# ZihaoW123/UniMM

Hardware: AMD Instinct MI355X
Metric: dialog-sequences/sec (fwd+bwd) at bs=240 seq=256 regions=36(+1 <IMG>) (higher is better)
Workload: dtype bf16; 1 GPU; UniMM-UL sparse training step (BASELINE configs[1]): bert_base_6layer_6conect, sequences_per_image=6, num_negative_samples=5, mask_prob=0.15, dropout on, MLM+UL / NSP / region-KL losses, fwd+bwd, optimizer step not included; global_batch=240, per_gpu_batch=240, seq_len=256, regions=37, parallelism=dp1, executor=eager launches, step_api=loss = combine(losses); loss.backward() (autograd, as train.py:164-168, :315)

## Files before the change

### include/unimm_hip.h

```cpp
#ifndef UNIMM_HIP_H
#define UNIMM_HIP_H

#include <stdint.h>

#ifdef __cplusplus
extern "C" {
#endif

#define UNIMM_OK 0
#define UNIMM_E_ARG (-1)
#define UNIMM_E_SHAPE (-2)
#define UNIMM_E_ALIGN (-3)
#define UNIMM_E_HIP (-4)

int unimm_version(void);
const char* unimm_arch(void);

enum {
  UNIMM_EPI_BIAS = 0,
  UNIMM_EPI_BIAS_GELU = 1,
  UNIMM_EPI_BIAS_DROP_RESID = 2,
  UNIMM_EPI_BIAS_RELU = 3,
  UNIMM_EPI_DGELU = 4,
  UNIMM_EPI_ADD = 5,
// ... 61 lines not shown
  const int32_t* order;
} unimm_attn_args;

int unimm_attn_fwd(const unimm_attn_args* args, void* stream);

int unimm_attn_probs(const unimm_attn_args* args, float* probs, void* stream);

typedef struct {
  const void* q; const void* k; const void* v; const void* out; const void* dout;
  const float* lse; float* delta;
  void* dq; void* dk; void* dv;
  const uint32_t* mask;
  const int32_t* q_off; const int32_t* q_len; const int32_t* k_off; const int32_t* k_len;
  int32_t B, H, Tq, Tk, D;
  int32_t ldq, ldk, ldv, ldo, lddo, lddq, lddk, lddv;
  int32_t mask_q_stride, mask_b_stride;
  float scale;
  uint32_t drop_key, drop_thr; float drop_scale;
  const uint32_t* drop_salt;
  const int32_t* order;
} unimm_attn_bwd_args;

int unimm_attn_bwd(const unimm_attn_bwd_args* args, void* stream);

enum { UNIMM_DT_U8 = 0, UNIMM_DT_I32 = 1, UNIMM_DT_I64 = 2, UNIMM_DT_F32 = 3 };

int unimm_mask_pack(const void* mask, int dtype, uint32_t* out, int64_t rows, int32_t t, void* stream);
int unimm_host_mask_pack(const void* mask, int dtype, uint32_t* out, int64_t rows, int32_t t, int32_t threads);
int unimm_host_memcpy(void* dst, const void* src, int64_t bytes, int32_t threads);
int unimm_mask_synth(const int32_t* mode, const int32_t* len, const int32_t* nans, uint32_t* text_words, uint32_t* co_words,
                     int32_t B, int32_t T, void* stream);

int unimm_plan_lengths(const uint32_t* text_words, int32_t t_q_stride, int32_t t_b_stride, const uint32_t* co_words,
                       int32_t c_q_stride, int32_t c_b_stride, int32_t R, const int32_t* labels, const int32_t* weights,
                       const float* nsp_weight, const int32_t* image_label, int32_t B, int32_t T, int32_t* header,
                       void* stream);
int unimm_plan_build(const int32_t* header, const int32_t* labels, const int32_t* weights, int32_t B, int32_t T,
                     int32_t* off, int32_t* lens, int64_t* rows, int64_t* inv, int32_t* lm_pos, int32_t* lm_idx,
                     int32_t* lm_label, int32_t* lm_weight, int32_t rows_cap, int32_t lm_cap, int32_t* dims_i, float* dims_f,
                     int32_t* order, void* stream);

int unimm_layernorm_fwd(const float* x, const float* gamma, const float* beta, float* y32, void* y16, float* mean,
                        float* rstd, int32_t M, int32_t H, float eps, uint32_t drop_key, uint32_t drop_thr,
                        float drop_scale, const uint32_t* drop_salt, void* stream);

int64_t unimm_colpartials_bytes(int32_t H);
// ... 210 lines not shown
```

### unimm_amd/csrc/api.hip

```cpp
#include "common.h"

extern "C" int unimm_version(void) { return 19; }
extern "C" const char* unimm_arch(void) { return "gfx950"; }
```

### unimm_amd/csrc/attention.hip

```cpp
#include <type_traits>
#include "common.h"

namespace {

struct AttnParams {
  const bf16_t* q; const bf16_t* k; const bf16_t* v;
  bf16_t* o; float* lse;
  const uint32_t* mask;
  const int* q_off; const int* q_len; const int* k_off; const int* k_len;
  const int* ks_off; const int* ks_len; int ks_ins;
  const int* order;
  int B, H, Tq, Tk, ldq, ldk, ldv, ldo;
  int mask_q_stride, mask_b_stride;
  int parts;
  float scale;
  DropoutArg drop;
};

constexpr float LOG2E = 1.4426950408889634f;
constexpr float LN2 = 0.6931471805599453f;

template <int D> __device__ __forceinline__ int swz(int row) {
  if constexpr (D == 64) { const int t = row >> 1; return (t & 7) ^ ((t & 1) << 2); }
  else return ((row & 3) << 2) | ((row >> 2) & 3);
// ... 58 lines not shown

__device__ __forceinline__ bf16x8 pack8(const float* p) {
  typedef __attribute__((ext_vector_type(4))) unsigned int u4;
  u4 w = {pack2bf(p[0], p[1]), pack2bf(p[2], p[3]), pack2bf(p[4], p[5]), pack2bf(p[6], p[7])};
  return __builtin_bit_cast(bf16x8, w);
}

__device__ __forceinline__ int key_of_reg(int reg, int h) { return (reg & 3) + 8 * (reg >> 2) + 4 * h; }

template <int D>
__device__ __forceinline__ void store_acc_row(bf16_t* __restrict__ g, const f32x16 (&a)[D / 32], float s, int h, bool ok) {
#pragma unroll
  for (int dt = 0; dt < D / 32; ++dt)
#pragma unroll
    for (int qp = 0; qp < 2; ++qp) {
      const uint32_t a0 = pack2bf(a[dt][8 * qp] * s, a[dt][8 * qp + 1] * s), a1 = pack2bf(a[dt][8 * qp + 2] * s, a[dt][8 * qp + 3] * s);
      const uint32_t b0 = pack2bf(a[dt][8 * qp + 4] * s, a[dt][8 * qp + 5] * s), b1 = pack2bf(a[dt][8 * qp + 6] * s, a[dt][8 * qp + 7] * s);
      const auto w0 = __builtin_amdgcn_permlane32_swap(a0, b0, false, false);
      const auto w1 = __builtin_amdgcn_permlane32_swap(a1, b1, false, false);
      if (ok) *reinterpret_cast<u32x4*>(g + 32 * dt + 16 * qp + 8 * h) = u32x4{w0[0], w1[0], w0[1], w1[1]};
    }
}

template <int D, int NKT>
__global__ __launch_bounds__(512, 2) void attn_fwd_kernel(AttnParams p) {
  drop_resolve(p.drop);
  extern __shared__ __attribute__((aligned(16))) char smem[];
  constexpr int KPAD = NKT * 32;
  char* kimg = smem;
  char* vimg = smem + KPAD * 2 * D;
  const int tid = threadIdx.x, wave = tid >> 6, lane = tid & 63;
  const int item = blockIdx.x / p.parts, part = blockIdx.x % p.parts;
  const int b = p.order != nullptr ? p.order[item / p.H] : item / p.H, head = item % p.H;
  const int nwv = blockDim.x >> 6;
  const int r = lane & 31, h = lane >> 5;

  const int Ts_b = p.ks_len ? p.ks_len[b] : 0;
  int Tk_b = (p.k_len ? p.k_len[b] : p.Tk) + Ts_b;
  Tk_b = Tk_b < KPAD ? Tk_b : KPAD;
  const int Tq_b = p.q_len ? p.q_len[b] : p.Tq;
  if (part * (int)(blockDim.x >> 6) * 32 >= Tq_b) return;
  const size_t qbase = p.q_off ? (size_t)p.q_off[b] : (size_t)b * p.Tq;
  const size_t kbase = p.k_off ? (size_t)p.k_off[b] : (size_t)b * p.Tk;
  const size_t sbase = p.ks_off ? (size_t)p.ks_off[b] : 0;
  const int kpad_b = ((Tk_b + 31) & ~31) < KPAD ? ((Tk_b + 31) & ~31) : KPAD;
  stage_head_seg<D>(p.k + head * D, p.ldk, kbase, sbase, p.ks_ins, Ts_b, Tk_b, kpad_b, kimg, tid, blockDim.x);
  stage_head_seg<D>(p.v + head * D, p.ldv, kbase, sbase, p.ks_ins, Ts_b, Tk_b, kpad_b, vimg, tid, blockDim.x);

  int wt = part * nwv + wave;
  int q0, qrow;
  bool qvalid;
  bf16x8 qf[D / 16];
  uint32_t mw[NKT];
#define UNIMM_LOAD_QTILE()                                                                                    \
  {                                                                                                          \
    q0 = wt * 32;                                                                                            \
    qrow = q0 + r;                                                                                           \
    qvalid = qrow < Tq_b;                                                                                    \
    if (!qvalid) qrow = Tq_b - 1;                                                                            \
    const bf16_t* qg_ = p.q + (qbase + qrow) * p.ldq + head * D;                                             \
    _Pragma("unroll") for (int ks = 0; ks < D / 16; ++ks) qf[ks] = *reinterpret_cast<const bf16x8*>(qg_ + 16 * ks + 8 * h); \
    const uint32_t* mp_ = p.mask + (size_t)b * p.mask_b_stride + (size_t)qrow * p.mask_q_stride;            \
    _Pragma("unroll") for (int t = 0; t < NKT; ++t) mw[t] = 32 * t < p.Tk ? mp_[t] : 0u;    \
  }
  UNIMM_LOAD_QTILE()
  stage_wait();
  __syncthreads();
  constexpr bool WALK = D == 64;
  for (bool first = true; wt * 32 < Tq_b && (WALK || first); first = false, wt += nwv * p.parts) {
    if (WALK && !first) UNIMM_LOAD_QTILE()

  f32x16 s[NKT];
#pragma unroll
  for (int t = 0; t < NKT; ++t) {
    f32x16 acc = {};
    if (32 * t < Tk_b) {
#pragma unroll
      for (int ks = 0; ks < D / 16; ++ks) {
        const bf16x8 kf = read_row_frag<D>(kimg, 32 * t + r, 2 * ks + h);
        acc = __builtin_amdgcn_mfma_f32_32x32x16_bf16(kf, qf[ks], acc, 0, 0, 0);
      }
    }
    s[t] = acc;
  }

  const float c1 = p.scale * LOG2E;
  constexpr float MOFF = -10000.0f * LOG2E;
  int tk_here = Tk_b;
  asm volatile("" : "+v"(tk_here));
  float mx = -INFINITY;
// ... 56 lines not shown
  for (int dt = 0; dt < D / 32; ++dt) o[dt] = f32x16{};
#pragma unroll
  for (int t = 0; t < NKT; ++t) {
    if (32 * t >= Tk_b) continue;
#pragma unroll
    for (int ss = 0; ss < 2; ++ss) {
      float pv[8];
#pragma unroll
      for (int j = 0; j < 8; ++j) pv[j] = s[t][8 * ss + j];
      const bf16x8 pf = pack8(pv);
#pragma unroll
      for (int dt = 0; dt < D / 32; ++dt) {
        const bf16x8 vf = read_tr_frag<D>(vimg, 32 * t + 16 * ss, 32 * dt, lane);
        o[dt] = __builtin_amdgcn_mfma_f32_32x32x16_bf16(vf, pf, o[dt], 0, 0, 0);
      }
    }
  }

  store_acc_row<D>(p.o + (qbase + (qvalid ? qrow : 0)) * p.ldo + head * D, o, inv, h, qvalid);
  if (qvalid) {
    if (p.lse != nullptr && h == 0) p.lse[((size_t)b * p.H + head) * p.Tq + qrow] = (mx + __log2f(sum)) * LN2;
  }
  }
#undef UNIMM_LOAD_QTILE
}


struct AttnBwdParams {
  const bf16_t* q; const bf16_t* k; const bf16_t* v; const bf16_t* o; const bf16_t* dout;
  const float* lse; float* delta;
  bf16_t* dq; bf16_t* dk; bf16_t* dv;
  const uint32_t* mask;
  const int* q_off; const int* q_len; const int* k_off; const int* k_len;
  const int* order;
  int B, H, Tq, Tk, ldq, ldk, ldv, ldo, lddo, lddq, lddk, lddv;
  int mask_q_stride, mask_b_stride;
  int parts;
  float scale;
  DropoutArg drop;
};

template <int D, int NKT>
__global__ __launch_bounds__(512, 2) void attn_bwd_dq_kernel(AttnBwdParams p) {
  drop_resolve(p.drop);
  extern __shared__ __attribute__((aligned(16))) char smem[];
  constexpr int KPAD = NKT * 32;
// ... 517 lines not shown
        const u32x2 hi = *reinterpret_cast<const u32x2*>(tile + r * 64 + (((4 * ss + 2 + h) ^ tile64_swz(r)) << 3));
        const bf16x8 pf = __builtin_bit_cast(bf16x8, u32x4{lo[0], lo[1], hi[0], hi[1]});
        const bf16x8 vf = read_tr_frag<D>(vimg, 32 * t + 16 * ss, 32 * dt, lane);
        o1[0] = __builtin_amdgcn_mfma_f32_32x32x16_bf16(vf, pf, o1[0], 0, 0, 0);
      }
    }
    float mx = -INFINITY, sum = 0.f;
#pragma unroll
    for (int w = 0; w < NW; ++w) {
      mx = fmaxf(mx, mx_w[w * QPAD + 32 * qt2 + r]);
      sum += sm_w[w * QPAD + 32 * qt2 + r];
    }
    const float inv = (p.drop.thr != 0u ? p.drop.scale : 1.0f) / sum;
    const int q = 32 * qt2 + r;
    const bool qvalid = q < Tq_b;
    store_acc_row<32>(p.o + (qbase + (qvalid ? q : 0)) * p.ldo + head * D + 32 * dt, o1, inv, h, qvalid);
    if (dt == 0 && qvalid && h == 0 && p.lse != nullptr) p.lse[((size_t)b * p.H + head) * p.Tq + q] = (mx + __log2f(sum)) * LN2;
  }
}

template <int NQT>
__global__ __launch_bounds__(512, 2) void attn_bwd_fused_kernel(AttnBwdParams p) {
  constexpr int D = 64;
  drop_resolve(p.drop);
  extern __shared__ __attribute__((aligned(16))) char smem[];
  constexpr int QPAD = NQT * 32;
  constexpr int AS = D + 4;
  char* qimg = smem;
  char* doimg = smem + QPAD * 2 * D;
  float* lse_s = reinterpret_cast<float*>(smem + 2 * QPAD * 2 * D);
  float* del_s = lse_s + QPAD;
  uint32_t* mw_s = reinterpret_cast<uint32_t*>(del_s + QPAD);
  char* scr = reinterpret_cast<char*>(mw_s + 8 * QPAD);
  float* acc = reinterpret_cast<float*>(scr + 8 * 2048);
  int* turn = reinterpret_cast<int*>(acc + QPAD * AS);
  const int tid = threadIdx.x, wave = tid >> 6, lane = tid & 63;
  const int item = blockIdx.x;
  const int b = p.order != nullptr ? p.order[item / p.H] : item / p.H, head = item % p.H;
  const int wt = wave;
  const int r = lane & 31, h = lane >> 5;

  const int Tq_b = p.q_len ? p.q_len[b] : p.Tq, Tk_b = p.k_len ? p.k_len[b] : p.Tk;
  const size_t qbase = p.q_off ? (size_t)p.q_off[b] : (size_t)b * p.Tq;
  const size_t kbase = p.k_off ? (size_t)p.k_off[b] : (size_t)b * p.Tk;
  const int qpad_b = ((Tq_b + 31) & ~31) < QPAD ? ((Tq_b + 31) & ~31) : QPAD;
  stage_head<D>(p.q + qbase * p.ldq + head * D, p.ldq, Tq_b, qpad_b, qimg, tid, blockDim.x);
// ... 10 lines not shown
  const bf16_t* vg = p.v + grow * p.ldv + head * D;
  bf16x8 kf[D / 16], vf[D / 16];
#pragma unroll
  for (int ks = 0; ks < D / 16; ++ks) {
    kf[ks] = *reinterpret_cast<const bf16x8*>(kg + 16 * ks + 8 * h);
    vf[ks] = *reinterpret_cast<const bf16x8*>(vg + 16 * ks + 8 * h);
  }
  bf16x8 ktf[2][2];
  {
    char* kt = reinterpret_cast<char*>(acc) + wave * (32 * 2 * D);
#pragma unroll
    for (int ks = 0; ks < D / 16; ++ks) {
      const u32x4 v = kvalid ? __builtin_bit_cast(u32x4, kf[ks]) : u32x4{0u, 0u, 0u, 0u};
      *reinterpret_cast<u32x4*>(kt + r * (2 * D) + (((2 * ks + h) ^ swz<D>(r)) << 4)) = v;
    }
#pragma unroll
    for (int ss = 0; ss < 2; ++ss) {
      ktf[0][ss] = read_tr_frag<D>(kt, 16 * ss, 0, lane);
      ktf[1][ss] = read_tr_frag<D>(kt, 16 * ss, 32, lane);
    }
  }
  stage_wait();
  __syncthreads();

  f32x16 dk[D / 32], dv[D / 32];
#pragma unroll
  for (int dt = 0; dt < D / 32; ++dt) { dk[dt] = f32x16{}; dv[dt] = f32x16{}; }
  const uint32_t* mrow = mw_s + wt * QPAD;
  char* ws = scr + wave * 2048;
  const uint32_t hbase = ((uint32_t)b * p.H + head) * (uint32_t)p.Tq;
  const uint32_t halfw = ((uint32_t)p.Tk + 1u) >> 1, halfm = halfw * DROP_M1;
  const uint32_t dlane = drop_lin(p.drop, (4u * (uint32_t)h + ((uint32_t)r & 1u)) * halfw + ((uint32_t)(wt * 32 + r) >> 1));
  const float c1 = p.scale * LOG2E;
  const bool dropping = p.drop.thr != 0u;
  const uint32_t thr16 = dropping ? (p.drop.thr >> 16) : 0u;
  const float dsc = dropping ? p.drop.scale : 1.0f;
  const BwdScoreCtx sctx{dlane, hbase, halfm, thr16, dsc, c1, dropping};

  if (wave_on) {
#pragma unroll 1
  for (int qt = 0; qt < NQT; ++qt) {
    if (32 * qt >= Tq_b) break;
    f32x16 sacc = {}, dpacc = {};
#pragma unroll
    for (int ks = 0; ks < D / 16; ++ks) {
      const bf16x8 qf = read_row_frag<D>(qimg, 32 * qt + r, 2 * ks + h);
// ... 34 lines not shown
        for (int g = 0; g < 4; ++g)
          *reinterpret_cast<f32x4*>(ap + 32 * dt + 8 * g) = f32x4{dqp[dt][4 * g], dqp[dt][4 * g + 1], dqp[dt][4 * g + 2], dqp[dt][4 * g + 3]};
    } else {
      while (__hip_atomic_load(turn + qt, __ATOMIC_ACQUIRE, __HIP_MEMORY_SCOPE_WORKGROUP) != wt) __builtin_amdgcn_s_sleep(2);
#pragma unroll
      for (int dt = 0; dt < 2; ++dt)
#pragma unroll
        for (int g = 0; g < 4; ++g) {
          f32x4* a4 = reinterpret_cast<f32x4*>(ap + 32 * dt + 8 * g);
          const f32x4 o = *a4;
          *a4 = f32x4{o[0] + dqp[dt][4 * g], o[1] + dqp[dt][4 * g + 1], o[2] + dqp[dt][4 * g + 2], o[3] + dqp[dt][4 * g + 3]};
        }
    }
    if (lane == 0) __hip_atomic_store(turn + qt, wt + 1, __ATOMIC_RELEASE, __HIP_MEMORY_SCOPE_WORKGROUP);
  }
  }

  if (wave_on) {
    const bool ok = kvalid;
    store_acc_row<D>(p.dk + (ok ? grow : 0) * p.lddk + head * D, dk, p.scale, h, ok);
    store_acc_row<D>(p.dv + (ok ? grow : 0) * p.lddv + head * D, dv, 1.0f, h, ok);
  }
  __syncthreads();
  for (int i = tid; i < qpad_b * 8; i += blockDim.x) {
    const int q = i >> 3, c = i & 7;
    if (q >= Tq_b) continue;
    float v[8];
#pragma unroll
    for (int j = 0; j < 8; ++j) v[j] = acc[q * AS + 8 * c + j] * p.scale;
    *reinterpret_cast<u32x4*>(p.dq + (qbase + q) * p.lddq + head * D + 8 * c) =
        u32x4{pack2bf(v[0], v[1]), pack2bf(v[2], v[3]), pack2bf(v[4], v[5]), pack2bf(v[6], v[7])};
  }
}

template <int NQT>
__global__ __launch_bounds__(512, 2) void attn_bwd_fewq128_kernel(AttnBwdParams p) {
  constexpr int D = 128;
  static_assert(NQT == 2, "the (sequence, head) item's queries are two 32-row tiles: P / dS of both stay in registers for phase 2");
  drop_resolve(p.drop);
  extern __shared__ __attribute__((aligned(16))) char smem[];
  constexpr int QPAD = NQT * 32;
  char* qimg = smem;
  char* doimg = smem + QPAD * 2 * D;
  float* lse_s = reinterpret_cast<float*>(smem + 2 * QPAD * 2 * D);
  float* del_s = lse_s + QPAD;
  uint32_t* mw_s = reinterpret_cast<uint32_t*>(del_s + QPAD);
  char* scr = reinterpret_cast<char*>(mw_s + 8 * QPAD);
  char* kimgs = scr + 8 * NQT * 2048;
  const int tid = threadIdx.x, wave = tid >> 6, lane = tid & 63;
  const int item = blockIdx.x;
  const int b = p.order != nullptr ? p.order[item / p.H] : item / p.H, head = item % p.H;
  const int wt = wave;
  const int r = lane & 31, h = lane >> 5;

// ... 313 lines not shown
    }
  }
  auto kern = attn_bwd_dkv_kernel<D, NQT>;
  if (set_lds(kern, lds) != UNIMM_OK) return UNIMM_E_HIP;
  hipLaunchKernelGGL(kern, dim3(p.B * p.H * q.parts), dim3(block_threads((tiles + q.parts - 1) / q.parts, NQT * 32)), lds, s, q);
  UNIMM_CHECK_LAUNCH();
  return UNIMM_OK;
}

template <int NQT>
int launch_bwd_fused(const AttnBwdParams& p, hipStream_t s) {
  constexpr int D = 64, QPAD = NQT * 32;
  const size_t lds = (size_t)2 * QPAD * 2 * D + 2 * QPAD * sizeof(float) + (size_t)8 * QPAD * sizeof(uint32_t) + 8 * 2048 +
                     (size_t)QPAD * (D + 4) * sizeof(float) + NQT * sizeof(int);
  auto kern = attn_bwd_fused_kernel<NQT>;
  if (set_lds(kern, lds) != UNIMM_OK) return UNIMM_E_HIP;
  AttnBwdParams q = p;
  q.parts = 1;
  hipLaunchKernelGGL(kern, dim3(p.B * p.H), dim3(512), lds, s, q);
  UNIMM_CHECK_LAUNCH();
  return UNIMM_OK;
}

inline int launch_bwd_fewq128(const AttnBwdParams& p, hipStream_t s) {
  constexpr int D = 128, NQT = 2, QPAD = NQT * 32;
  const size_t lds = (size_t)2 * QPAD * 2 * D + 2 * QPAD * sizeof(float) + (size_t)8 * QPAD * sizeof(uint32_t) + 8 * NQT * 2048 +
                     (size_t)8 * 32 * 2 * D;
  auto kern = attn_bwd_fewq128_kernel<NQT>;
  if (set_lds(kern, lds) != UNIMM_OK) return UNIMM_E_HIP;
  AttnBwdParams q = p;
  q.parts = 1;
  hipLaunchKernelGGL(kern, dim3(p.B * p.H), dim3(512), lds, s, q);
  UNIMM_CHECK_LAUNCH();
  return UNIMM_OK;
}

inline int launch_bwd_fewk128(const AttnBwdParams& p, hipStream_t s) {
  constexpr int D = 128, KPAD = 64, QMAX = 256;
  const size_t lds = (size_t)2 * KPAD * 2 * D + 2 * QMAX * sizeof(float) + (size_t)2 * QMAX * sizeof(uint32_t) + 8 * 6144 +
                     (size_t)2 * (QMAX / 32) * 2 * 2 * 1024;
  auto kern = attn_bwd_fewk128_kernel;
  if (set_lds(kern, lds) != UNIMM_OK) return UNIMM_E_HIP;
  AttnBwdParams q = p;
  q.parts = 1;
  hipLaunchKernelGGL(kern, dim3(p.B * p.H), dim3(512), lds, s, q);
  UNIMM_CHECK_LAUNCH();
// ... 69 lines not shown
  }
#pragma unroll
  for (int o = 32; o > 0; o >>= 1) mx = fmaxf(mx, __shfl_xor(mx, o, 64));
  float sum = 0.f;
#pragma unroll
  for (int j = 0; j < 4; ++j) {
    sc[j] = (lane + 64 * j) < p.Tk ? __expf(sc[j] - mx) : 0.f;
    sum += sc[j];
  }
  sum = wave_sum(sum);
  const float inv = 1.0f / sum;
  float* out = probs + (size_t)row * p.Tk;
#pragma unroll
  for (int j = 0; j < 4; ++j) {
    const int key = lane + 64 * j;
    if (key >= p.Tk) continue;
    float v = sc[j] * inv;
    if (p.drop.thr != 0u) v = drop_apply(p.drop, (uint32_t)row, (uint32_t)p.Tk, (uint32_t)key, v);
    out[key] = v;
  }
}

}

extern "C" int unimm_attn_fwd(const unimm_attn_args* a, void* stream) {
  if (a == nullptr || !a->q || !a->k || !a->v || !a->out || !a->mask) return UNIMM_E_ARG;
  if (a->B <= 0 || a->H <= 0 || a->Tq <= 0 || a->Tk <= 0 || a->Tq > 256 || a->Tk > 256) return UNIMM_E_SHAPE;
  if (a->D != 64 && a->D != 128) return UNIMM_E_SHAPE;
  if ((a->ldq % 8) || (a->ldk % 8) || (a->ldv % 8) || (a->ldo % 8)) return UNIMM_E_ALIGN;
  if (((uintptr_t)a->q | (uintptr_t)a->k | (uintptr_t)a->v | (uintptr_t)a->out) & 15) return UNIMM_E_ALIGN;
  AttnParams p;
  p.q = (const bf16_t*)a->q; p.k = (const bf16_t*)a->k; p.v = (const bf16_t*)a->v;
  p.o = (bf16_t*)a->out; p.lse = a->lse; p.mask = a->mask;
  p.q_off = a->q_off; p.q_len = a->q_len; p.k_off = a->k_off; p.k_len = a->k_len;
  if ((p.q_off == nullptr) != (p.q_len == nullptr) || (p.k_off == nullptr) != (p.k_len == nullptr)) return UNIMM_E_ARG;
  p.ks_off = a->ks_off; p.ks_len = a->ks_len; p.ks_ins = a->ks_ins;
  if ((p.ks_off == nullptr) != (p.ks_len == nullptr)) return UNIMM_E_ARG;
  if (p.ks_off != nullptr && (p.k_off == nullptr || a->ks_ins < 0 || a->drop_thr != 0u)) return UNIMM_E_ARG;
  if (p.ks_off == nullptr) p.ks_ins = 0;
  p.order = a->order;
  p.B = a->B; p.H = a->H; p.Tq = a->Tq; p.Tk = a->Tk;
  p.ldq = a->ldq; p.ldk = a->ldk; p.ldv = a->ldv; p.ldo = a->ldo;
  p.mask_q_stride = a->mask_q_stride; p.mask_b_stride = a->mask_b_stride;
  p.scale = a->scale;
  p.drop.key = a->drop_key; p.drop.thr = a->drop_thr; p.drop.scale = a->drop_scale; p.drop.salt = a->drop_salt;
  hipStream_t s = (hipStream_t)stream;
// ... 34 lines not shown
  if (a->B <= 0 || a->H <= 0 || a->Tq <= 0 || a->Tk <= 0 || a->Tq > 256 || a->Tk > 256) return UNIMM_E_SHAPE;
  if (a->D != 64 && a->D != 128) return UNIMM_E_SHAPE;
  if ((a->ldq % 8) || (a->ldk % 8) || (a->ldv % 8) || (a->ldo % 8) || (a->lddo % 8) || (a->lddq % 8) || (a->lddk % 8) ||
      (a->lddv % 8))
    return UNIMM_E_ALIGN;
  if (((uintptr_t)a->q | (uintptr_t)a->k | (uintptr_t)a->v | (uintptr_t)a->out | (uintptr_t)a->dout | (uintptr_t)a->dq |
       (uintptr_t)a->dk | (uintptr_t)a->dv) & 15)
    return UNIMM_E_ALIGN;
  AttnBwdParams p;
  p.q = (const bf16_t*)a->q; p.k = (const bf16_t*)a->k; p.v = (const bf16_t*)a->v; p.o = (const bf16_t*)a->out;
  p.dout = (const bf16_t*)a->dout; p.lse = a->lse; p.delta = a->delta;
  p.dq = (bf16_t*)a->dq; p.dk = (bf16_t*)a->dk; p.dv = (bf16_t*)a->dv; p.mask = a->mask;
  p.q_off = a->q_off; p.q_len = a->q_len; p.k_off = a->k_off; p.k_len = a->k_len;
  if ((p.q_off == nullptr) != (p.q_len == nullptr) || (p.k_off == nullptr) != (p.k_len == nullptr)) return UNIMM_E_ARG;
  p.order = a->order;
  p.B = a->B; p.H = a->H; p.Tq = a->Tq; p.Tk = a->Tk;
  p.ldq = a->ldq; p.ldk = a->ldk; p.ldv = a->ldv; p.ldo = a->ldo; p.lddo = a->lddo;
  p.lddq = a->lddq; p.lddk = a->lddk; p.lddv = a->lddv;
  p.mask_q_stride = a->mask_q_stride; p.mask_b_stride = a->mask_b_stride;
  p.scale = a->scale;
  p.drop.key = a->drop_key; p.drop.thr = a->drop_thr; p.drop.scale = a->drop_scale; p.drop.salt = a->drop_salt;
  hipStream_t s = (hipStream_t)stream;
  const bool small_k = a->Tk <= 64, small_q = a->Tq <= 64;
  if (a->D == 64 && !small_k && !small_q) return launch_bwd_fused<8>(p, s);
#ifndef UNIMM_ATTN_FEWQ128
#define UNIMM_ATTN_FEWQ128 1
#endif
  if (UNIMM_ATTN_FEWQ128 && a->D == 128 && small_q && !small_k) return launch_bwd_fewq128(p, s);
#ifndef UNIMM_ATTN_FEWK128
#define UNIMM_ATTN_FEWK128 1
#endif
  if (UNIMM_ATTN_FEWK128 && a->D == 128 && small_k && !small_q) return launch_bwd_fewk128(p, s);
  int rc;
  if (a->D == 64) rc = small_k ? launch_bwd_dq<64, 2>(p, s) : launch_bwd_dq<64, 8>(p, s);
  else rc = small_k ? launch_bwd_dq<128, 2>(p, s) : launch_bwd_dq<128, 8>(p, s);
  if (rc != UNIMM_OK) return rc;
  if (a->D == 64) return small_q ? launch_bwd_dkv<64, 2>(p, s) : launch_bwd_dkv<64, 8>(p, s);
  return small_q ? launch_bwd_dkv<128, 2>(p, s) : launch_bwd_dkv<128, 8>(p, s);
}
```

### unimm_amd/lib.py

```python
from __future__ import annotations

import ctypes as C
import os
import threading

import torch

_PKG = os.path.dirname(os.path.abspath(__file__))
LIB_PATH = os.path.join(_PKG, "libunimm_hip.so")
ABI_VERSION = 19

EPI_BIAS, EPI_BIAS_GELU, EPI_BIAS_DROP_RESID, EPI_BIAS_RELU, EPI_DGELU, EPI_ADD, EPI_MUL, EPI_BIAS_GELU_DG = range(8)

_ERR = {-1: "UNIMM_E_ARG", -2: "UNIMM_E_SHAPE", -3: "UNIMM_E_ALIGN", -4: "UNIMM_E_HIP"}


class UnimmHipError(RuntimeError):
    pass


class GemmNtArgs(C.Structure):
    _fields_ = [("x", C.c_void_p), ("w", C.c_void_p), ("bias", C.c_void_p), ("aux", C.c_void_p),
                ("out", C.c_void_p), ("out2", C.c_void_p),
                ("M", C.c_int32), ("N", C.c_int32), ("K", C.c_int32),
                ("ldx", C.c_int32), ("ldw", C.c_int32), ("ldaux", C.c_int32), ("ldo", C.c_int32),
                ("epilogue", C.c_int32), ("out_f32", C.c_int32),
                ("drop_key", C.c_uint32), ("drop_thr", C.c_uint32), ("drop_scale", C.c_float),
                ("aux_mean", C.c_void_p), ("aux_rstd", C.c_void_p), ("aux_gamma", C.c_void_p), ("aux_beta", C.c_void_p),
                ("tile", C.c_int32), ("drop_salt", C.c_void_p),
                ("splitk_ws", C.c_void_p), ("splitk_ws_bytes", C.c_int64), ("splitk", C.c_int32)]


class GemmTnArgs(C.Structure):
# ... 37 lines not shown
    L.unimm_kv_cache_update.argtypes = [VP, VP]
    L.unimm_lm_topk.argtypes = [VP, I32, I32, I32, VP, I32, VP, I32, I32, VP, VP, VP, VP]
    L.unimm_gemm_tn_grouped.argtypes = [VP, I32, VP]
    L.unimm_gemm_tn_grouped_ws.argtypes = [VP, I32, I32, VP, I64, VP]
    L.unimm_colpartials_finish_grouped.argtypes = [VP, I32, VP]
    L.unimm_layernorm_fwd.argtypes = [VP] * 7 + [I32, I32, F32, U32, U32, F32, VP, VP]
    L.unimm_x3_layernorm_fwd.argtypes = [VP] * 7 + [I32, I32, F32, U32, U32, F32, VP, VP]
    L.unimm_layernorm_bwd_partials.argtypes = [VP] * 8 + [I32, I32, U32, U32, F32, U32, U32, F32, VP, VP, VP, VP]
    L.unimm_layernorm_bwd.argtypes = [VP] * 11 + [I32, I32, U32, U32, F32, U32, U32, F32, VP, VP]
    _lib = L
    return L


SYMBOLS = ["unimm_version", "unimm_arch", "unimm_gemm_nt", "unimm_gemm_tn", "unimm_gemm_tn_grouped", "unimm_attn_fwd", "unimm_attn_bwd",
           "unimm_mask_pack", "unimm_layernorm_fwd", "unimm_colpartials_bytes", "unimm_layernorm_bwd",
           "unimm_embed_fwd", "unimm_embed_bwd", "unimm_colsum", "unimm_cast_f32_bf16", "unimm_transpose_cast",
           "unimm_pack_image", "unimm_mul_dropout", "unimm_mul_dropout_bwd", "unimm_lm_loss_fwd",
           "unimm_lm_loss_bwd", "unimm_kl_loss_fwd", "unimm_kl_loss_bwd", "unimm_nsp_loss_fwd",
           "unimm_nsp_loss_bwd", "unimm_reduce_sum", "unimm_segment_sum", "unimm_gelu_bwd", "unimm_gather_rows", "unimm_prof_enable", "unimm_prof_collect", "unimm_adamw_step", "unimm_transpose_cast_grouped", "unimm_mask_synth", "unimm_neural_ndcg", "unimm_plan_lengths", "unimm_plan_build", "unimm_layernorm_bwd_partials",
           "unimm_colpartials_finish_grouped", "unimm_gemm_tn_grouped_ws", "unimm_linear_f32", "unimm_rows_add_f32", "unimm_transpose_bf16", "unimm_sum_slabs_bf16", "unimm_attn_probs",
           "unimm_x3_split", "unimm_x3_split_wt", "unimm_x3_layernorm_bwd_partials", "unimm_embed_bwd_f32", "unimm_x3_lm_loss_bwd",
           "unimm_x3_kl_loss_bwd", "unimm_x3_rows_add", "unimm_x3_attn_fwd", "unimm_x3_attn_bwd", "unimm_x3_attn_set_impl", "unimm_x3_layernorm_fwd", "unimm_prof_tag", "unimm_prof_tagged",
           "unimm_sum_dropout", "unimm_sum_dropout_bwd", "unimm_mse_loss_fwd", "unimm_mse_loss_bwd", "unimm_host_mask_pack", "unimm_host_memcpy",
           "unimm_attn_decode", "unimm_kv_cache_update", "unimm_lm_topk"]


def _check(rc, what):
    if rc != 0:
        raise UnimmHipError(f"{what} failed: {_ERR.get(rc, rc)}")


_tls = threading.local()


def scoped_stream():
    return getattr(_tls, "stream", None)


def _stream():
    s = getattr(_tls, "stream", None)
    if s is not None:
        return s
    return C.c_void_p(torch.cuda.current_stream().cuda_stream)


class stream_scope:

# ... 799 lines not shown
                drop=NO_DROP, qvar=None, kvar=None, planes=None):
    _dev(q, k, v, out, dout, lse, delta, dq, dk, dv, mask)
    a = AttnBwdArgs()
    pl = None
    if planes is not None:
        pl = X3AttnPlanes()
        pl.dq3, pl.dk3, pl.dv3, pl.cp3, pl.ld3 = dq.data_ptr(), dk.data_ptr(), dv.data_ptr(), planes[0], planes[1]
    a.q_off, a.q_len = (qvar[0].data_ptr(), qvar[1].data_ptr()) if qvar is not None else (None, None)
    a.k_off, a.k_len = (kvar[0].data_ptr(), kvar[1].data_ptr()) if kvar is not None else (None, None)
    a.order = _item_order(qvar, kvar)
    a.q, a.k, a.v, a.out, a.dout = q.data_ptr(), k.data_ptr(), v.data_ptr(), out.data_ptr(), dout.data_ptr()
    a.lse, a.delta, a.mask = lse.data_ptr(), delta.data_ptr(), mask.data_ptr()
    if pl is None:
        a.dq, a.dk, a.dv = dq.data_ptr(), dk.data_ptr(), dv.data_ptr()
        a.lddq, a.lddk, a.lddv = dq.stride(0), dk.stride(0), dv.stride(0)
    a.B, a.H, a.Tq, a.Tk, a.D = B, H, Tq, Tk, D
    a.ldq, a.ldk, a.ldv, a.ldo, a.lddo = q.stride(0), k.stride(0), v.stride(0), out.stride(0), dout.stride(0)
    a.mask_q_stride, a.mask_b_stride, a.scale = mask_q_stride, mask_b_stride, scale
    a.drop_key, a.drop_thr, a.drop_scale = drop[:3]
    a.drop_salt = _salt(drop)
    _check(lib().unimm_x3_attn_bwd(C.byref(a), C.byref(pl) if pl is not None else None, _stream()), "unimm_x3_attn_bwd")


def x3_attn_set_impl(impl):
    _check(lib().unimm_x3_attn_set_impl(int(impl)), "unimm_x3_attn_set_impl")


def x3_layernorm_fwd(x, gamma, beta, y32, y3, mean, rstd, M, H, eps=1e-12, drop=NO_DROP):
    _dev(x, gamma, beta, y32, y3, mean, rstd)
    _check(lib().unimm_x3_layernorm_fwd(x.data_ptr(), gamma.data_ptr(), beta.data_ptr(), _P(y32), y3.data_ptr(), _P(mean), _P(rstd),
                                        M, H, eps, drop[0], drop[1], drop[2], _salt(drop), _stream()), "unimm_x3_layernorm_fwd")
```

Baseline: 6040 dialog-sequences/sec.

## Add persistent attention-backward kernel with cross-item staging overlap

Adds a persistent D=64 attention backward kernel that launches one workgroup per CU and walks (batch, head) items in a serpentine order to balance variable-length sequences. When the current item leaves waves idle and the LDS budget allows, those idle waves stage the next item's Q/dO tiles, row stats and mask into a second LDS slot. The dQ reduction across waves uses ordered LDS accumulation guarded by per-tile turn flags instead of a separate pass. The new path is the default and replaces the fused per-item launch. It adds spin-waiting and LDS pressure, and trace stamps compiled in only under a debug macro.

Measured after the change: 6062 dialog-sequences/sec (median of 4 runs). About the same (+0.4%).

```diff
diff --git a/include/unimm_hip.h b/include/unimm_hip.h
--- a/include/unimm_hip.h
+++ b/include/unimm_hip.h
@@ -107,6 +107,7 @@
 } unimm_attn_bwd_args;
 
 int unimm_attn_bwd(const unimm_attn_bwd_args* args, void* stream);
+int unimm_attn_set_impl(int32_t impl);
 
 enum { UNIMM_DT_U8 = 0, UNIMM_DT_I32 = 1, UNIMM_DT_I64 = 2, UNIMM_DT_F32 = 3 };
 
diff --git a/unimm_amd/csrc/api.hip b/unimm_amd/csrc/api.hip
--- a/unimm_amd/csrc/api.hip
+++ b/unimm_amd/csrc/api.hip
@@ -1,4 +1,4 @@
 #include "common.h"
 
-extern "C" int unimm_version(void) { return 19; }
+extern "C" int unimm_version(void) { return 20; }
 extern "C" const char* unimm_arch(void) { return "gfx950"; }
diff --git a/unimm_amd/csrc/attention.hip b/unimm_amd/csrc/attention.hip
--- a/unimm_amd/csrc/attention.hip
+++ b/unimm_amd/csrc/attention.hip
@@ -104,9 +104,31 @@
     }
 }
 
+#ifdef UNIMM_ATTN_TRACE
+__device__ unsigned long long* g_attn_trace = nullptr;
+#define UNIMM_ATTN_STAMP(slot)                                                                          \
+  if (g_attn_trace != nullptr && threadIdx.x == 0) g_attn_trace[(size_t)blockIdx.x * 8 + (slot)] = wall_clock64();
+#define UNIMM_ATTN_STAMP_ID(seq, len)                                                                   \
+  if (g_attn_trace != nullptr && threadIdx.x == 0) {                                                   \
+    g_attn_trace[(size_t)blockIdx.x * 8 + 4] = (unsigned long long)__builtin_amdgcn_s_getreg(4 | (0 << 6) | (31 << 11));   \
+    g_attn_trace[(size_t)blockIdx.x * 8 + 5] = (unsigned long long)(seq);                              \
+    g_attn_trace[(size_t)blockIdx.x * 8 + 6] = (unsigned long long)(len);                              \
+    g_attn_trace[(size_t)blockIdx.x * 8 + 7] = (unsigned long long)__builtin_amdgcn_s_getreg(6164);    \
+  }
+#define UNIMM_ATTN_STAMP_DRAIN() __builtin_amdgcn_s_waitcnt(0x0F70);
+#define UNIMM_ATTN_STAMP_ITEM(item, slot, thread)                                                       \
+  if (g_attn_trace != nullptr && threadIdx.x == (thread)) g_attn_trace[(size_t)(item) * 8 + (slot)] = wall_clock64();
+#else
+#define UNIMM_ATTN_STAMP(slot)
+#define UNIMM_ATTN_STAMP_ITEM(item, slot, thread)
+#define UNIMM_ATTN_STAMP_DRAIN()
+#define UNIMM_ATTN_STAMP_ID(seq, len)
+#endif
+
 template <int D, int NKT>
 __global__ __launch_bounds__(512, 2) void attn_fwd_kernel(AttnParams p) {
   drop_resolve(p.drop);
+  UNIMM_ATTN_STAMP(0)
   extern __shared__ __attribute__((aligned(16))) char smem[];
   constexpr int KPAD = NKT * 32;
   char* kimg = smem;
@@ -148,6 +170,8 @@
   UNIMM_LOAD_QTILE()
   stage_wait();
   __syncthreads();
+  UNIMM_ATTN_STAMP(1)
+  UNIMM_ATTN_STAMP_ID(b, Tk_b)
   constexpr bool WALK = D == 64;
   for (bool first = true; wt * 32 < Tq_b && (WALK || first); first = false, wt += nwv * p.parts) {
     if (WALK && !first) UNIMM_LOAD_QTILE()
@@ -250,6 +274,9 @@
     if (p.lse != nullptr && h == 0) p.lse[((size_t)b * p.H + head) * p.Tq + qrow] = (mx + __log2f(sum)) * LN2;
   }
   }
+  UNIMM_ATTN_STAMP(2)
+  UNIMM_ATTN_STAMP_DRAIN()
+  UNIMM_ATTN_STAMP(3)
 #undef UNIMM_LOAD_QTILE
 }
 
@@ -813,6 +840,7 @@
 template <int NQT>
 __global__ __launch_bounds__(512, 2) void attn_bwd_fused_kernel(AttnBwdParams p) {
   constexpr int D = 64;
+  UNIMM_ATTN_STAMP(0)
   drop_resolve(p.drop);
   extern __shared__ __attribute__((aligned(16))) char smem[];
   constexpr int QPAD = NQT * 32;
@@ -869,6 +897,8 @@
   }
   stage_wait();
   __syncthreads();
+  UNIMM_ATTN_STAMP(1)
+  UNIMM_ATTN_STAMP_ID(b, Tq_b)
 
   f32x16 dk[D / 32], dv[D / 32];
 #pragma unroll
@@ -949,6 +979,7 @@
     store_acc_row<D>(p.dv + (ok ? grow : 0) * p.lddv + head * D, dv, 1.0f, h, ok);
   }
   __syncthreads();
+  UNIMM_ATTN_STAMP(2)
   for (int i = tid; i < qpad_b * 8; i += blockDim.x) {
     const int q = i >> 3, c = i & 7;
     if (q >= Tq_b) continue;
@@ -957,6 +988,313 @@
     for (int j = 0; j < 8; ++j) v[j] = acc[q * AS + 8 * c + j] * p.scale;
     *reinterpret_cast<u32x4*>(p.dq + (qbase + q) * p.lddq + head * D + 8 * c) =
         u32x4{pack2bf(v[0], v[1]), pack2bf(v[2], v[3]), pack2bf(v[4], v[5]), pack2bf(v[6], v[7])};
+  }
+  UNIMM_ATTN_STAMP_DRAIN()
+  UNIMM_ATTN_STAMP(3)
+}
+
+constexpr int PB_TOP = 160 * 1024;
+constexpr int PB_SCR = 8 * 2048;
+constexpr int PB_LO = PB_SCR + 2 * 8 * (int)sizeof(int);
+constexpr int PB_SET = 2 * 2 * 64 + 2 * (int)sizeof(float) + 8 * (int)sizeof(uint32_t);
+constexpr int PB_ACC = (64 + 4) * (int)sizeof(float);
+__host__ __device__ inline bool pb_pair_fits(int p_cur, int p_next) {
+  return PB_LO + (PB_SET + PB_ACC) * p_cur + PB_SET * p_next <= PB_TOP;
+}
+static_assert(PB_LO + (PB_SET + PB_ACC) * 256 <= PB_TOP, "a 256-row item alone must fit");
+
+struct PbItem {
+  int b, head, Tq_b, Tk_b, qpad;
+  size_t qbase, kbase;
+};
+__device__ __forceinline__ PbItem pb_item(const AttnBwdParams& p, int item) {
+  PbItem it;
+  it.b = p.order != nullptr ? p.order[item / p.H] : item / p.H;
+  it.head = item % p.H;
+  it.Tq_b = p.q_len ? p.q_len[it.b] : p.Tq;
+  it.Tk_b = p.k_len ? p.k_len[it.b] : p.Tk;
+  it.qbase = p.q_off ? (size_t)p.q_off[it.b] : (size_t)it.b * p.Tq;
+  it.kbase = p.k_off ? (size_t)p.k_off[it.b] : (size_t)it.b * p.Tk;
+  it.qpad = ((it.Tq_b + 31) & ~31) < 256 ? ((it.Tq_b + 31) & ~31) : 256;
+  return it;
+}
+struct PbLds {
+  char* qimg; char* doimg;
+  float* lse_s; float* del_s;
+  uint32_t* mw_s;
+  float* acc;
+};
+__device__ __forceinline__ PbLds pb_carve(char* smem, int slot, int P) {
+  char* set = slot == 0 ? smem + PB_LO : smem + PB_TOP - PB_SET * P;
+  PbLds l;
+  l.qimg = set;
+  l.doimg = set + P * 128;
+  l.lse_s = reinterpret_cast<float*>(set + P * 256);
+  l.del_s = l.lse_s + P;
+  l.mw_s = reinterpret_cast<uint32_t*>(l.del_s + P);
+  l.acc = reinterpret_cast<float*>(slot == 0 ? set + PB_SET * P : set - PB_ACC * P);
+  return l;
+}
+__device__ __forceinline__ void pb_row_stats(const AttnBwdParams& p, const PbItem& it, const PbLds& l, int tid, int nthreads) {
+  constexpr int D = 64, LPR = 8, NB = 4;
+  const int P = it.qpad, Tq_b = it.Tq_b, Tk_b = it.Tk_b;
+  {
+    float v[NB];
+    const size_t stat = ((size_t)it.b * p.H + it.head) * p.Tq;
+#pragma unroll
+    for (int u = 0; u < NB; ++u) {
+      const int i = tid + u * nthreads;
+      v[u] = i < Tq_b ? p.lse[stat + i] : 0.f;
+    }
+#pragma unroll
+    for (int u = 0; u < NB; ++u) {
+      const int i = tid + u * nthreads;
+      if (i < P) l.lse_s[i] = i < Tq_b ? -v[u] * LOG2E : -INFINITY;
+    }
+  }
+  for (int base = tid; base < P * LPR; base += NB * nthreads) {
+    u32x4 a[NB], o[NB];
+#pragma unroll
+    for (int u = 0; u < NB; ++u) {
+      const int i = base + u * nthreads, row = i / LPR, c = i % LPR;
+      a[u] = u32x4{0u, 0u, 0u, 0u}; o[u] = u32x4{0u, 0u, 0u, 0u};
+      if (i < P * LPR && row < Tq_b) {
+        a[u] = *reinterpret_cast<const u32x4*>(p.dout + (it.qbase + row) * p.lddo + it.head * D + 8 * c);
+        o[u] = *reinterpret_cast<const u32x4*>(p.o + (it.qbase + row) * p.ldo + it.head * D + 8 * c);
+      }
+    }
+#pragma unroll
+    for (int u = 0; u < NB; ++u) {
+      const int i = base + u * nthreads, row = i / LPR, c = i % LPR;
+      if (i >= P * LPR) break;
+      float part = 0.f;
+      if (row < Tq_b) {
+#pragma unroll
+        for (int e = 0; e < 4; ++e) {
+          part = fmaf(__uint_as_float(a[u][e] << 16), __uint_as_float(o[u][e] << 16), part);
+          part = fmaf(__uint_as_float(a[u][e] & 0xffff0000u), __uint_as_float(o[u][e] & 0xffff0000u), part);
+        }
+      }
+#pragma unroll
+      for (int x = 1; x < LPR; x <<= 1) part += __shfl_xor(part, x, 64);
+      if (c == 0) l.del_s[row] = part;
+    }
+  }
+  const int nkt_b = (Tk_b + 31) >> 5;
+  const uint32_t* mb = p.mask + (size_t)it.b * p.mask_b_stride;
+  constexpr int MB = 8;
+  for (int base = tid; base < nkt_b * P; base += MB * nthreads) {
+    uint32_t w[MB];
+#pragma unroll
+    for (int u = 0; u < MB; ++u) {
+      const int i = base + u * nthreads;
+      const int kt = i / P, qi = i - kt * P;
+      const int qc = qi < Tq_b ? qi : Tq_b - 1;
+      w[u] = i < nkt_b * P ? mb[(size_t)qc * p.mask_q_stride + kt] : 0u;
+    }
+#pragma unroll
+    for (int u = 0; u < MB; ++u) {
+      const int i = base + u * nthreads;
+      const int kt = i / P, qi = i - kt * P;
+      if (i < nkt_b * P) l.mw_s[kt * P + qi] = ~w[u] | pad_key_bits(Tk_b, kt);
+    }
+  }
+}
+__device__ __forceinline__ void pb_stage(const AttnBwdParams& p, const PbItem& it, const PbLds& l, int tid, int nthreads) {
+  stage_head<64>(p.q + it.qbase * p.ldq + it.head * 64, p.ldq, it.Tq_b, it.qpad, l.qimg, tid, nthreads);
+  stage_head<64>(p.dout + it.qbase * p.lddo + it.head * 64, p.lddo, it.Tq_b, it.qpad, l.doimg, tid, nthreads);
+  pb_row_stats(p, it, l, tid, nthreads);
+}
+__device__ __forceinline__ void pb_load_kv(const AttnBwdParams& p, const PbItem& it, int wt, int r, int h, bf16x8 (&kf)[4], bf16x8 (&vf)[4]) {
+  int krow = wt * 32 + r;
+  if (krow >= it.Tk_b) krow = it.Tk_b - 1;
+  const bf16_t* kg = p.k + (it.kbase + krow) * p.ldk + it.head * 64;
+  const bf16_t* vg = p.v + (it.kbase + krow) * p.ldv + it.head * 64;
+#pragma unroll
+  for (int ks = 0; ks < 4; ++ks) {
+    kf[ks] = *reinterpret_cast<const bf16x8*>(kg + 16 * ks + 8 * h);
+    vf[ks] = *reinterpret_cast<const bf16x8*>(vg + 16 * ks + 8 * h);
+  }
+}
+
+__global__ __launch_bounds__(512, 2) void attn_bwd_pers_kernel(AttnBwdParams p) {
+  constexpr int D = 64, AS = D + 4;
+  drop_resolve(p.drop);
+  extern __shared__ __attribute__((aligned(16))) char smem[];
+  char* scr = smem;
+  int* turn_all = reinterpret_cast<int*>(smem + PB_SCR);
+  const int tid = threadIdx.x, wave = tid >> 6, lane = tid & 63;
+  const int wt = wave;
+  const int r = lane & 31, h = lane >> 5;
+  char* ws = scr + wave * 2048;
+  const int nitems = p.B * p.H;
+  const float c1 = p.scale * LOG2E;
+  const bool dropping = p.drop.thr != 0u;
+  const uint32_t thr16 = dropping ? (p.drop.thr >> 16) : 0u;
+  const float dsc = dropping ? p.drop.scale : 1.0f;
+  const uint32_t halfw = ((uint32_t)p.Tk + 1u) >> 1, halfm = halfw * DROP_M1;
+
+  const int grid = (int)gridDim.x, wg = (int)blockIdx.x;
+  const int nfull = nitems / grid;
+  const int n_mine = nfull + (((nfull & 1) ? grid - 1 - wg : wg) < nitems - nfull * grid ? 1 : 0);
+  auto item_at = [&](int j) {
+    const int st = (j & 1) ? n_mine - ((j + 1) >> 1) : (j >> 1);
+    return st * grid + ((st & 1) ? grid - 1 - wg : wg);
+  };
+  int visit = 0, item = item_at(0), slot = 0;
+  bf16x8 kf[D / 16], vf[D / 16];
+  {
+    const PbItem it0 = pb_item(p, item);
+    pb_stage(p, it0, pb_carve(smem, slot, it0.qpad), tid, 512);
+    if (tid < 16) turn_all[tid] = 0;
+    pb_load_kv(p, it0, wt, r, h, kf, vf);
+    stage_wait();
+    __syncthreads();
+  }
+
+  for (;;) {
+    UNIMM_ATTN_STAMP_ITEM(item, 0, 0)
+    const PbItem cur = pb_item(p, item);
+    const PbLds L = pb_carve(smem, slot, cur.qpad);
+    const bool has_next = visit + 1 < n_mine;
+    const int nkt = (cur.Tk_b + 31) >> 5;
+    const int Tq_b = cur.Tq_b, Tk_b = cur.Tk_b, head = cur.head, P = cur.qpad;
+    const bool kvalid = wt * 32 + r < Tk_b;
+    const bool wave_on = wt * 32 < Tk_b;
+    const size_t grow = cur.kbase + (kvalid ? wt * 32 + r : Tk_b - 1);
+    int* turn = turn_all + 8 * slot;
+
+    bf16x8 ktf[2][2];
+    uint32_t dlane;
+    {
+      int tid1 = tid;
+      asm volatile("" : "+v"(tid1));
+      const int lane1 = tid1 & 63, r1 = tid1 & 31, h1 = (tid1 >> 5) & 1;
+      dlane = drop_lin(p.drop, (4u * (uint32_t)h1 + ((uint32_t)r1 & 1u)) * halfw + ((uint32_t)((tid1 >> 6) * 32 + r1) >> 1));
+      char* ws1 = scr + (tid1 >> 6) * 2048;
+#pragma unroll
+      for (int ss = 0; ss < 2; ++ss) {
+        if ((r1 >> 4) == ss) {
+#pragma unroll
+          for (int ks = 0; ks < D / 16; ++ks) {
+            const u32x4 v = kvalid ? __builtin_bit_cast(u32x4, kf[ks]) : u32x4{0u, 0u, 0u, 0u};
+            *reinterpret_cast<u32x4*>(ws1 + (r1 & 15) * (2 * D) + (((2 * ks + h1) ^ swz<D>(r1)) << 4)) = v;
+          }
+        }
+        ktf[0][ss] = read_tr_frag<D>(ws1, 0, 0, lane1);
+        ktf[1][ss] = read_tr_frag<D>(ws1, 0, 32, lane1);
+      }
+    }
+
+    f32x16 dk[D / 32], dv[D / 32];
+#pragma unroll
+    for (int dt = 0; dt < D / 32; ++dt) { dk[dt] = f32x16{}; dv[dt] = f32x16{}; }
+    const uint32_t* mrow = L.mw_s + wt * P;
+    const uint32_t hbase = ((uint32_t)cur.b * p.H + head) * (uint32_t)p.Tq;
+    const BwdScoreCtx sctx{dlane, hbase, halfm, thr16, dsc, c1, dropping};
+
+    if (wave_on) {
+#pragma unroll 1
+      for (int qt = 0; qt < 8; ++qt) {
+        if (32 * qt >= Tq_b) break;
+        f32x16 sacc = {}, dpacc = {};
+#pragma unroll
+        for (int ks = 0; ks < D / 16; ++ks) {
+          const bf16x8 qf = read_row_frag<D>(L.qimg, 32 * qt + r, 2 * ks + h);
+          sacc = __builtin_amdgcn_mfma_f32_32x32x16_bf16(qf, kf[ks], sacc, 0, 0, 0);
+          const bf16x8 df = read_row_frag<D>(L.doimg, 32 * qt + r, 2 * ks + h);
+          dpacc = __builtin_amdgcn_mfma_f32_32x32x16_bf16(df, vf[ks], dpacc, 0, 0, 0);
+        }
+        float pd[16], ds[16];
+        bwd_score_tile(p, sctx, sacc, dpacc, L.lse_s, L.del_s, mrow, 32 * qt, r, h, pd, ds);
+#pragma unroll
+        for (int g4 = 0; g4 < 4; ++g4)
+          *reinterpret_cast<u32x2*>(ws + r * 64 + (((2 * g4 + h) ^ tile64_swz(r)) << 3)) =
+              u32x2{pack2bf(ds[4 * g4], ds[4 * g4 + 1]), pack2bf(ds[4 * g4 + 2], ds[4 * g4 + 3])};
+#pragma unroll
+        for (int ss = 0; ss < 2; ++ss) {
+          const bf16x8 pf = pack8(pd + 8 * ss);
+          const bf16x8 dsf = pack8(ds + 8 * ss);
+#pragma unroll
+          for (int dt = 0; dt < D / 32; ++dt) {
+            const bf16x8 dotf = read_tr_frag<D>(L.doimg, 32 * qt + 16 * ss, 32 * dt, lane);
+            dv[dt] = __builtin_amdgcn_mfma_f32_32x32x16_bf16(dotf, pf, dv[dt], 0, 0, 0);
+            const bf16x8 qtf = read_tr_frag<D>(L.qimg, 32 * qt + 16 * ss, 32 * dt, lane);
+            dk[dt] = __builtin_amdgcn_mfma_f32_32x32x16_bf16(qtf, dsf, dk[dt], 0, 0, 0);
+          }
+        }
+        f32x16 dqp[2] = {f32x16{}, f32x16{}};
+#pragma unroll
+        for (int ss = 0; ss < 2; ++ss) {
+          const bf16x8 dstf = read_tr_tile64s(ws, 16 * ss, lane);
+          dqp[0] = __builtin_amdgcn_mfma_f32_32x32x16_bf16(ktf[0][ss], dstf, dqp[0], 0, 0, 0);
+          dqp[1] = __builtin_amdgcn_mfma_f32_32x32x16_bf16(ktf[1][ss], dstf, dqp[1], 0, 0, 0);
+        }
+        float* ap = L.acc + (32 * qt + r) * AS + 4 * h;
+        if (wt == 0) {
+#pragma unroll
+          for (int dt = 0; dt < 2; ++dt)
+#pragma unroll
+            for (int g = 0; g < 4; ++g)
+              *reinterpret_cast<f32x4*>(ap + 32 * dt + 8 * g) = f32x4{dqp[dt][4 * g], dqp[dt][4 * g + 1], dqp[dt][4 * g + 2], dqp[dt][4 * g + 3]};
+        } else {
+          while (__hip_atomic_load(turn + qt, __ATOMIC_ACQUIRE, __HIP_MEMORY_SCOPE_WORKGROUP) != wt) __builtin_amdgcn_s_sleep(2);
+#pragma unroll
+          for (int dt = 0; dt < 2; ++dt)
+#pragma unroll
+            for (int g = 0; g < 4; ++g) {
+              f32x4* a4 = reinterpret_cast<f32x4*>(ap + 32 * dt + 8 * g);
+              const f32x4 o = *a4;
+              *a4 = f32x4{o[0] + dqp[dt][4 * g], o[1] + dqp[dt][4 * g + 1], o[2] + dqp[dt][4 * g + 2], o[3] + dqp[dt][4 * g + 3]};
+            }
+        }
+        if (lane == 0) __hip_atomic_store(turn + qt, wt + 1, __ATOMIC_RELEASE, __HIP_MEMORY_SCOPE_WORKGROUP);
+      }
+      store_acc_row<D>(p.dk + (kvalid ? grow : 0) * p.lddk + head * D, dk, p.scale, h, kvalid);
+      store_acc_row<D>(p.dv + (kvalid ? grow : 0) * p.lddv + head * D, dv, 1.0f, h, kvalid);
+    }
+    UNIMM_ATTN_STAMP_ITEM(item, 1, 0)
+    int tid2 = tid;
+    asm volatile("" : "+v"(tid2));
+    bool piped = false;
+    if (has_next) {
+      int nxt_here = item_at(visit + 1);
+      asm volatile("" : "+s"(nxt_here));
+      const PbItem nx = pb_item(p, nxt_here);
+      piped = nkt < 8 && pb_pair_fits(P, nx.qpad);
+      if (piped && !wave_on) pb_stage(p, nx, pb_carve(smem, slot ^ 1, nx.qpad), tid2 - nkt * 64, (8 - nkt) * 64);
+      pb_load_kv(p, nx, tid2 >> 6, tid2 & 31, (tid2 >> 5) & 1, kf, vf);
+      if (piped && !wave_on) stage_wait();
+      if (piped && !wave_on) { UNIMM_ATTN_STAMP_ITEM(item, 4, 448) }
+    }
+    __syncthreads();
+    UNIMM_ATTN_STAMP_ITEM(item, 2, 0)
+    if (tid2 < 8) turn[tid2] = 0;
+    for (int i = tid2; i < P * 8; i += 512) {
+      const int q = i >> 3, c = i & 7;
+      if (q >= Tq_b) continue;
+      float v[8];
+#pragma unroll
+      for (int j = 0; j < 8; ++j) v[j] = L.acc[q * AS + 8 * c + j] * p.scale;
+      *reinterpret_cast<u32x4*>(p.dq + (cur.qbase + q) * p.lddq + head * D + 8 * c) =
+          u32x4{pack2bf(v[0], v[1]), pack2bf(v[2], v[3]), pack2bf(v[4], v[5]), pack2bf(v[6], v[7])};
+    }
+#ifdef UNIMM_ATTN_TRACE
+    if (g_attn_trace != nullptr && tid == 0) { g_attn_trace[(size_t)item * 8 + 6] = (unsigned long long)Tq_b; g_attn_trace[(size_t)item * 8 + 5] = blockIdx.x; }
+    if (!has_next) { UNIMM_ATTN_STAMP_ITEM(item, 3, 0) }
+#endif
+    if (!has_next) break;
+    __syncthreads();
+    const int item_done = item;
+    item = item_at(++visit); slot ^= 1;
+    if (!piped) {
+      const PbItem nx = pb_item(p, item);
+      pb_stage(p, nx, pb_carve(smem, slot, nx.qpad), tid2, 512);
+      stage_wait();
+      __syncthreads();
+    }
+    UNIMM_ATTN_STAMP_ITEM(item_done, 3, 0)
+    (void)item_done;
   }
 }
 
@@ -1316,6 +1654,26 @@
   return UNIMM_OK;
 }
 
+int g_attn_impl = 1;
+
+inline int launch_bwd_pers(const AttnBwdParams& p, hipStream_t s) {
+  static int n_cu = 0;
+  if (n_cu == 0) {
+    int dev = 0;
+    hipDeviceProp_t prop;
+    if (hipGetDevice(&dev) != hipSuccess || hipGetDeviceProperties(&prop, dev) != hipSuccess || prop.multiProcessorCount <= 0) return UNIMM_E_HIP;
+    n_cu = prop.multiProcessorCount;
+  }
+  auto kern = attn_bwd_pers_kernel;
+  if (set_lds(kern, PB_TOP) != UNIMM_OK) return UNIMM_E_HIP;
+  AttnBwdParams q = p;
+  q.parts = 1;
+  const int items = p.B * p.H;
+  hipLaunchKernelGGL(kern, dim3(items < n_cu ? items : n_cu), dim3(512), PB_TOP, s, q);
+  UNIMM_CHECK_LAUNCH();
+  return UNIMM_OK;
+}
+
 inline int launch_bwd_fewq128(const AttnBwdParams& p, hipStream_t s) {
   constexpr int D = 128, NQT = 2, QPAD = NQT * 32;
   const size_t lds = (size_t)2 * QPAD * 2 * D + 2 * QPAD * sizeof(float) + (size_t)8 * QPAD * sizeof(uint32_t) + 8 * NQT * 2048 +
@@ -1431,6 +1789,18 @@
 }
 
 }
+
+extern "C" int unimm_attn_set_impl(int32_t impl) {
+  if (impl != 0 && impl != 1) return UNIMM_E_ARG;
+  g_attn_impl = impl;
+  return UNIMM_OK;
+}
+
+#ifdef UNIMM_ATTN_TRACE
+extern "C" int unimm_debug_attn_trace(void* buf) {
+  return hipMemcpyToSymbol(HIP_SYMBOL(g_attn_trace), &buf, sizeof(buf)) == hipSuccess ? 0 : 1;
+}
+#endif
 
 extern "C" int unimm_attn_fwd(const unimm_attn_args* a, void* stream) {
   if (a == nullptr || !a->q || !a->k || !a->v || !a->out || !a->mask) return UNIMM_E_ARG;
@@ -1511,7 +1881,7 @@
   p.drop.key = a->drop_key; p.drop.thr = a->drop_thr; p.drop.scale = a->drop_scale; p.drop.salt = a->drop_salt;
   hipStream_t s = (hipStream_t)stream;
   const bool small_k = a->Tk <= 64, small_q = a->Tq <= 64;
-  if (a->D == 64 && !small_k && !small_q) return launch_bwd_fused<8>(p, s);
+  if (a->D == 64 && !small_k && !small_q) return g_attn_impl == 1 ? launch_bwd_pers(p, s) : launch_bwd_fused<8>(p, s);
 #ifndef UNIMM_ATTN_FEWQ128
 #define UNIMM_ATTN_FEWQ128 1
 #endif
diff --git a/unimm_amd/lib.py b/unimm_amd/lib.py
--- a/unimm_amd/lib.py
+++ b/unimm_amd/lib.py
@@ -8,7 +8,7 @@
 
 _PKG = os.path.dirname(os.path.abspath(__file__))
 LIB_PATH = os.path.join(_PKG, "libunimm_hip.so")
-ABI_VERSION = 19
+ABI_VERSION = 20
 
 EPI_BIAS, EPI_BIAS_GELU, EPI_BIAS_DROP_RESID, EPI_BIAS_RELU, EPI_DGELU, EPI_ADD, EPI_MUL, EPI_BIAS_GELU_DG = range(8)
 
@@ -92,7 +92,8 @@
            "unimm_x3_split", "unimm_x3_split_wt", "unimm_x3_layernorm_bwd_partials", "unimm_embed_bwd_f32", "unimm_x3_lm_loss_bwd",
            "unimm_x3_kl_loss_bwd", "unimm_x3_rows_add", "unimm_x3_attn_fwd", "unimm_x3_attn_bwd", "unimm_x3_attn_set_impl", "unimm_x3_layernorm_fwd", "unimm_prof_tag", "unimm_prof_tagged",
            "unimm_sum_dropout", "unimm_sum_dropout_bwd", "unimm_mse_loss_fwd", "unimm_mse_loss_bwd", "unimm_host_mask_pack", "unimm_host_memcpy",
-           "unimm_attn_decode", "unimm_kv_cache_update", "unimm_lm_topk"]
+           "unimm_attn_decode", "unimm_kv_cache_update", "unimm_lm_topk",
+           "unimm_attn_set_impl"]
 
 
 def _check(rc, what):
@@ -938,6 +939,10 @@
     _check(lib().unimm_x3_attn_bwd(C.byref(a), C.byref(pl) if pl is not None else None, _stream()), "unimm_x3_attn_bwd")
 
 
+def attn_set_impl(impl):
+    _check(lib().unimm_attn_set_impl(int(impl)), "unimm_attn_set_impl")
+
+
 def x3_attn_set_impl(impl):
     _check(lib().unimm_x3_attn_set_impl(int(impl)), "unimm_x3_attn_set_impl")
 
```
